# AKGWSB/EzRT

Measured on NVIDIA H100. Metric: Mrays/s (primary+secondary), higher is better.
Workload: dtype f32

## Files before the change

### ezrt_b200/csrc/device_functions.cuh

```cuda
#ifndef EZRT_DEVICE_FUNCTIONS_CUH
#define EZRT_DEVICE_FUNCTIONS_CUH

#include "device_scene.h"
#include "ezrt.h"
#include "ezrt_math.h"
#include "w8_node.h"

__constant__ uint32_t c_sobolV[8 * 32] = {
#include "ezrt_sobol_table.inc"
};

typedef ez_vec3 vec3;

__device__ __forceinline__ vec3 f4xyz(float4 q) { return ez_v3(q.x, q.y, q.z); }
__device__ __forceinline__ vec3 splat3(float s) { return ez_v3(s, s, s); }
__device__ __forceinline__ float4 ldg4(const float4* p) { return __ldg(p); }

#ifndef EZRT_MATH_NOINLINE
#define EZRT_MATH_NOINLINE 0
#endif
#if EZRT_MATH_NOINLINE
#define EZD_MATH __device__ __noinline__
#else
#define EZD_MATH __device__ __forceinline__
// ... 1146 lines not shown
                const unsigned p = __ballot_sync(FULL, member && da[a] >= 0.0f);
                signs |= (p == members ? 1u : (p == 0u ? 2u : 0u)) << (2 * a);
                const float4 b = make_float4(warp_reduce_f<0>(member ? oa[a] : INFINITY), warp_reduce_f<1>(member ? oa[a] : -INFINITY),
                                             warp_reduce_f<0>(member ? va[a] : INFINITY), warp_reduce_f<1>(member ? va[a] : -INFINITY));
                bnd[a] = b;
            }
        }
        const uint32_t near_mask = __shfl_sync(FULL, (d.x >= 0.0f ? (1u << sc.w8_near_bit[0]) : 0u) | (d.y >= 0.0f ? (1u << sc.w8_near_bit[1]) : 0u) |
                                                         (d.z >= 0.0f ? (1u << sc.w8_near_bit[2]) : 0u), __ffs(members) - 1);
        float L = EZ_INF;
        int sp = 0;
        uint32_t node = 0, g_base = 0, g_bits = 0;
        while (true) {
            const uint4* nd = nodes + (size_t)node * (W8_NODE_WORDS / 4);
            const uint4 h = ldg128_u32(nd), c = ldg128_u32(nd + 1), l = ldg128_u32(nd + 2), m = ldg128_u32(nd + 3), u = ldg128_u32(nd + 4);
            if (COUNT && lane == 0) ++*s_visits;
            bool hit = false;
            if (lane < 8) {
                const float sx = __uint_as_float(W8_SCALE_BITS(h.w, 0)), sy = __uint_as_float(W8_SCALE_BITS(h.w, 1)), sz = __uint_as_float(W8_SCALE_BITS(h.w, 2));
                const float ox = __uint_as_float(h.x), oy = __uint_as_float(h.y), oz = __uint_as_float(h.z);
                float ex, ey, ez, xx, xy, xz;
                w8_bundle_axis(__fadd_rd(ox, (slot_byte(c.z, c.w) - 0.25f) * sx), __fadd_ru(ox, (slot_byte(m.z, m.w) + 0.25f) * sx), signs & 3u, bnd[0], ex, xx);
                w8_bundle_axis(__fadd_rd(oy, (slot_byte(l.x, l.y) - 0.25f) * sy), __fadd_ru(oy, (slot_byte(u.x, u.y) + 0.25f) * sy), (signs >> 2) & 3u, bnd[1], ey, xy);
                w8_bundle_axis(__fadd_rd(oz, (slot_byte(l.z, l.w) - 0.25f) * sz), __fadd_ru(oz, (slot_byte(u.z, u.w) + 0.25f) * sz), signs >> 4, bnd[2], ez, xz);
                hit = fmaxf(fmaxf(ex, ey), fmaxf(ez, 0.0f)) <= fminf(fminf(xx, xy), fminf(xz, L));
            }
            const uint32_t hits = __ballot_sync(FULL, hit) & 0xffu;
            const uint32_t imask = h.w >> 24;
            const uint32_t inner = hits & imask;
            uint32_t leaf = hits & ~imask;
            if ((g_bits >> 8) != 0u) stack[sp++] = make_uint2(g_base, g_bits);
            g_base = c.x;
            g_bits = imask | ((uint32_t)s_perm[near_mask * 256u + inner] << 8);
            uint32_t t_mask = 0u;
            while (leaf != 0u) {
                const int s = __ffs(leaf) - 1;
                leaf &= leaf - 1u;
                const uint32_t mb = ((s < 4 ? m.x : m.y) >> ((s & 3) * 8)) & 0xffu;
                t_mask |= ((1u << (mb >> 5)) - 1u) << (mb & 31u);
            }
            if (t_mask != 0u) {
                while (t_mask != 0u) {
                    const int tri = (int)c.y + __ffs(t_mask) - 1;
                    t_mask &= t_mask - 1u;
                    if (member) {
                        if (COUNT) n_tests++;
                        float t = 0.0f;
                        const int r = IDX ? tri_test_idx_t<true>(sc.acc_tri_geo + (size_t)tri * 2, sc.acc_tri_vert, o, d, best, t, tri_na)
                                          : tri_test_t<true>(sc.acc_tri_geo + (size_t)tri * 4, o, d, best, t, tri_na);
                        if (r == 2) tie = true;
                        else if (r == 1) { best = t; best_tri = tri; tie = false; }
                    }
                }
                const float slack = sc.prune_delta * fmaxf(ez_abs(inv.x), fmaxf(ez_abs(inv.y), ez_abs(inv.z)));
                const float lim = member ? best + (best * 0.000244140625f + slack) : 0.0f;
                L = __uint_as_float(__reduce_max_sync(FULL, __float_as_uint(lim)));
            }
            if ((g_bits >> 8) == 0u) {
                if (sp == 0) break;
                const uint2 e = stack[--sp];
                g_base = e.x;
                g_bits = e.y;
            }
            const int p = 23 - __clz(g_bits);
            g_bits ^= 0x100u << p;
            const uint32_t slot = (uint32_t)p ^ near_mask;
            node = g_base + (uint32_t)__popc(g_bits & 0xffu & ((1u << slot) - 1u));
        }
        if (member) {
            HitRec hr;
            hr.t = best;
            hr.tri = best_tri;
            io.store(idx, hr, tie, o, d, inv);
        }
        }
    }
    if (COUNT) {
        if (lane == 0) atomicAdd(counts.node_visits, (unsigned long long)*s_visits);
        atomicAdd(counts.tri_tests, (unsigned long long)n_tests);
    }
}

struct MaterialDev {
    vec3 emissive, baseColor;
    float subsurface, metallic, specular, specularTint, roughness, anisotropic, sheen, sheenTint, clearcoat,
        clearcoatGloss;
};

__device__ __forceinline__ MaterialDev load_material(const SceneDev& sc, int matId) {
    const float4* m = sc.materials + (size_t)matId * 5;
    float4 a = ldg4(m), b = ldg4(m + 1), c = ldg4(m + 2), d = ldg4(m + 3);
    MaterialDev r;
    r.emissive = ez_v3(a.x, a.y, a.z);
    r.baseColor = ez_v3(a.w, b.x, b.y);
    r.subsurface = b.z; r.metallic = b.w; r.specular = c.x; r.specularTint = c.y;
    r.roughness = c.z; r.anisotropic = c.w; r.sheen = d.x; r.sheenTint = d.y;
    r.clearcoat = d.z; r.clearcoatGloss = d.w;
    return r;
}
__device__ __forceinline__ vec3 load_emissive(const SceneDev& sc, int matId) {
    float4 a = ldg4(sc.materials + (size_t)matId * 5);
    return ez_v3(a.x, a.y, a.z);
}

struct SurfaceHit {
    vec3 P, N;
    int matId;
    bool inside;
};

__device__ __forceinline__ const float4* tri_geo_rec(const SceneDev& sc, int tri, bool accel_space) {
    return accel_space ? sc.acc_tri_geo + (size_t)tri * (sc.acc_tri_indexed ? 2 : 4) : sc.tri_geo + (size_t)tri * 4;
}
__device__ __forceinline__ SurfaceHit surface_hit(const SceneDev& sc, vec3 o, vec3 d, float t, int tri, bool p3fudge, bool accel_space = false) {
    const float4* g = tri_geo_rec(sc, tri, accel_space);
    const float4* v = g;
    uint32_t i1 = 1u, i2 = 2u, i3 = 3u;
    if (accel_space && sc.acc_tri_indexed) {
        const uint4 qi = __ldg(reinterpret_cast<const uint4*>(g + 1));
        v = sc.acc_tri_vert; i1 = qi.x; i2 = qi.y; i3 = qi.z;
    }
    float4 q0 = ldg4(g), q1 = ldg4(v + i1), q2 = ldg4(v + i2), q3 = ldg4(v + i3);
    const float4* s = (accel_space ? sc.acc_tri_shade : sc.tri_shade) + (size_t)tri * 3;
    float4 m0 = ldg4(s), m1 = ldg4(s + 1), m2 = ldg4(s + 2);
    vec3 p1 = f4xyz(q1), p2 = f4xyz(q2), p3 = f4xyz(q3);
    vec3 Ng = f4xyz(q0);
    bool inside = ez_dot(Ng, d) > 0.0f;
    vec3 P = ez_add(o, ez_scale(d, t));
    float alpha, beta;
    float an = (-(P.x - p2.x)) * (p3.y - p2.y) + (P.y - p2.y) * (p3.x - p2.x);
    float bn = (-(P.x - p3.x)) * (p1.y - p3.y) + (P.y - p3.y) * (p1.x - p3.x);
    if (!p3fudge) {
        alpha = EZ_DIV(an, ((-(p1.x - p2.x)) * (p3.y - p2.y) + (p1.y - p2.y) * (p3.x - p2.x)) + 1e-7f);
        beta = EZ_DIV(bn, ((-(p2.x - p3.x)) * (p1.y - p3.y) + (p2.y - p3.y) * (p1.x - p3.x)) + 1e-7f);
    } else {
        alpha = EZ_DIV(an, (-((p1.x - p2.x) - 0.00005f)) * ((p3.y - p2.y) + 0.00005f) +
                               ((p1.y - p2.y) + 0.00005f) * ((p3.x - p2.x) + 0.00005f));
        beta = EZ_DIV(bn, (-((p2.x - p3.x) - 0.00005f)) * ((p1.y - p3.y) + 0.00005f) +
                              ((p2.y - p3.y) + 0.00005f) * ((p1.x - p3.x) + 0.00005f));
    }
    float gama = (1.0f - alpha) - beta;
    vec3 Ns = ez_add(ez_add(ez_scale(f4xyz(m0), alpha), ez_scale(f4xyz(m1), beta)), ez_scale(f4xyz(m2), gama));
    Ns = ez_normalize(Ns);
    SurfaceHit r;
    r.P = P;
    r.N = inside ? ez_neg(Ns) : Ns;
    r.matId = __float_as_int(m0.w);
    r.inside = inside;
    return r;
}
__device__ __forceinline__ int tri_material(const SceneDev& sc, int tri) {
    return __float_as_int(ldg4(sc.tri_shade + (size_t)tri * 3).w);
}

__device__ __forceinline__ float SchlickFresnel(float u) {
    float m = ez_clamp(1.0f - u, 0.0f, 1.0f);
    float m2 = m * m;
    return m2 * m2 * m;
}
__device__ __forceinline__ float GTR1(float NdotH, float a) {
    if (a >= 1.0f) return EZ_DIV(1.0f, EZ_PI);
    float a2 = a * a;
    float t = 1.0f + (a2 - 1.0f) * NdotH * NdotH;
    return EZ_DIV(a2 - 1.0f, EZ_PI * ezd_log(a2) * t);
}
__device__ __forceinline__ float GTR2(float NdotH, float a) {
    float a2 = a * a;
    float t = 1.0f + (a2 - 1.0f) * NdotH * NdotH;
    return EZ_DIV(a2, EZ_PI * t * t);
}
__device__ __forceinline__ float GTR2_aniso(float NdotH, float HdotX, float HdotY, float ax, float ay) {
    float s = ez_sqr(EZ_DIV(HdotX, ax)) + ez_sqr(EZ_DIV(HdotY, ay)) + NdotH * NdotH;
    return EZ_DIV(1.0f, EZ_PI * ax * ay * ez_sqr(s));
}
__device__ __forceinline__ float smithG_GGX(float NdotV, float alphaG) {
    float a = alphaG * alphaG;
    float b = NdotV * NdotV;
    return EZ_DIV(1.0f, NdotV + EZ_SQRT(a + b - a * b));
}
__device__ __forceinline__ float smithG_GGX_aniso(float NdotV, float VdotX, float VdotY, float ax, float ay) {
    return EZ_DIV(1.0f, NdotV + EZ_SQRT(ez_sqr(VdotX * ax) + ez_sqr(VdotY * ay) + ez_sqr(NdotV)));
}
__device__ __forceinline__ void get_tangent(vec3 N, vec3& tangent, vec3& bitangent) {
    vec3 helper = ez_v3(1.0f, 0.0f, 0.0f);
    if (ez_abs(N.x) > 0.999f) helper = ez_v3(0.0f, 0.0f, 1.0f);
    bitangent = ez_normalize(ez_cross(N, helper));
    tangent = ez_normalize(ez_cross(N, bitangent));
}

template <bool ANISO>
__device__ __forceinline__ vec3 brdf_evaluate(vec3 V, vec3 N, vec3 L, const MaterialDev& mat) {
    float NdotL = ez_dot(N, L);
    float NdotV = ez_dot(N, V);
    if (NdotL < 0.0f || NdotV < 0.0f) return splat3(0.0f);

    vec3 H = ez_normalize(ez_add(L, V));
    float NdotH = ez_dot(N, H);
    float LdotH = ez_dot(L, H);

    vec3 Cdlin = mat.baseColor;
    float Cdlum = 0.3f * Cdlin.x + 0.6f * Cdlin.y + 0.1f * Cdlin.z;
    vec3 Ctint = (Cdlum > 0.0f) ? ez_divs(Cdlin, Cdlum) : splat3(1.0f);
    vec3 Cspec = ez_scale(ez_vmix(splat3(1.0f), Ctint, mat.specularTint), mat.specular);
    vec3 Cspec0 = ez_vmix(ez_scale(Cspec, 0.08f), Cdlin, mat.metallic);
    vec3 Csheen = ez_vmix(splat3(1.0f), Ctint, mat.sheenTint);

    float Fd90 = 0.5f + 2.0f * LdotH * LdotH * mat.roughness;
    float FL = SchlickFresnel(NdotL);
    float FV = SchlickFresnel(NdotV);
    float Fd = ez_mix(1.0f, Fd90, FL) * ez_mix(1.0f, Fd90, FV);

    float Fss90 = LdotH * LdotH * mat.roughness;
    float Fss = ez_mix(1.0f, Fss90, FL) * ez_mix(1.0f, Fss90, FV);
    float ss = 1.25f * (Fss * (EZ_DIV(1.0f, NdotL + NdotV) - 0.5f) + 0.5f);

    float Ds, Gs;
    float FH = SchlickFresnel(LdotH);
    vec3 Fs = ez_vmix(Cspec0, splat3(1.0f), FH);
    if (!ANISO) {
        float alpha = ez_max(0.001f, ez_sqr(mat.roughness));
        Ds = GTR2(NdotH, alpha);
        Gs = smithG_GGX(NdotL, mat.roughness);
        Gs *= smithG_GGX(NdotV, mat.roughness);
    } else {
        vec3 X, Y;
        get_tangent(N, X, Y);
        float aspect = EZ_SQRT(1.0f - mat.anisotropic * 0.9f);
        float ax = ez_max(0.001f, EZ_DIV(ez_sqr(mat.roughness), aspect));
        float ay = ez_max(0.001f, ez_sqr(mat.roughness) * aspect);
        Ds = GTR2_aniso(NdotH, ez_dot(H, X), ez_dot(H, Y), ax, ay);
        Gs = smithG_GGX_aniso(NdotL, ez_dot(L, X), ez_dot(L, Y), ax, ay);
        Gs *= smithG_GGX_aniso(NdotV, ez_dot(V, X), ez_dot(V, Y), ax, ay);
    }

    float Dr = GTR1(NdotH, ez_mix(0.1f, 0.001f, mat.clearcoatGloss));
    float Fr = ez_mix(0.04f, 1.0f, FH);
    float Gr = smithG_GGX(NdotL, 0.25f) * smithG_GGX(NdotV, 0.25f);

    vec3 Fsheen = ez_scale(Csheen, FH * mat.sheen);
    vec3 diffuse = ez_add(ez_scale(Cdlin, EZ_DIV(1.0f, EZ_PI) * ez_mix(Fd, ss, mat.subsurface)), Fsheen);
    vec3 specular = ez_scale(ez_scale(Fs, Gs), Ds);
    vec3 clearcoat = splat3(0.25f * Gr * Fr * Dr * mat.clearcoat);
    return ez_add(ez_add(ez_scale(diffuse, 1.0f - mat.metallic), specular), clearcoat);
}

__device__ __forceinline__ float brdf_pdf(vec3 V, vec3 N, vec3 L, const MaterialDev& mat) {
    float NdotL = ez_dot(N, L);
    float NdotV = ez_dot(N, V);
    if (NdotL < 0.0f || NdotV < 0.0f) return 0.0f;
    vec3 H = ez_normalize(ez_add(L, V));
    float NdotH = ez_dot(N, H);
    float alpha = ez_max(0.001f, ez_sqr(mat.roughness));
    float Ds = GTR2(NdotH, alpha);
    float Dr = GTR1(NdotH, ez_mix(0.1f, 0.001f, mat.clearcoatGloss));
    float LH4 = 4.0f * ez_dot(L, H);
    float pdf_diffuse = EZ_DIV(NdotL, EZ_PI);
    float pdf_specular = EZ_DIV(Ds * NdotH, LH4);
    float pdf_clearcoat = EZ_DIV(Dr * NdotH, LH4);
    float r_diffuse = 1.0f - mat.metallic;
    float r_specular = 1.0f;
    float r_clearcoat = 0.25f * mat.clearcoat;
    float r_sum = r_diffuse + r_specular + r_clearcoat;
    float p_diffuse = EZ_DIV(r_diffuse, r_sum);
    float p_specular = EZ_DIV(r_specular, r_sum);
    float p_clearcoat = EZ_DIV(r_clearcoat, r_sum);
    float pdf = p_diffuse * pdf_diffuse + p_specular * pdf_specular + p_clearcoat * pdf_clearcoat;
    return ez_max(1e-10f, pdf);
}
__device__ __forceinline__ float mis_mix_weight(float a, float b) {
    float t = a * a;
    return EZ_DIV(t, b * b + t);
}

struct TransLobe {
    float t, eta, alpha;
    bool matched;
};
__device__ __forceinline__ TransLobe trans_lobe(const SceneDev& sc, int matId, const MaterialDev& mat, bool inside) {
    const float4 e = ldg4(sc.materials + (size_t)matId * 5 + 4);
    TransLobe r;
    r.t = ez_trans_weight(e.y, mat.metallic, e.x);
    r.eta = ez_trans_eta(e.x, inside);
    r.alpha = ez_max(0.001f, ez_sqr(mat.roughness));
    r.matched = ez_trans_matched(e.x) != 0;
    return r;
}
__device__ __forceinline__ vec3 bsdf_evaluate(vec3 V, vec3 N, vec3 L, const MaterialDev& mat, const TransLobe& tl, float& pdf) {
    vec3 f_ref = splat3(0.0f), f_diel = splat3(0.0f);
    float pdf_ref = 0.0f, pdf_diel = 0.0f;
    if (ez_dot(N, L) > 0.0f) { f_ref = brdf_evaluate<false>(V, N, L, mat); pdf_ref = brdf_pdf(V, N, L, mat); }
    if (!tl.matched) f_diel = ez_diel_eval(V, N, L, mat.baseColor, tl.alpha, tl.eta, &pdf_diel);
    return ez_trans_mix(f_ref, pdf_ref, f_diel, pdf_diel, tl.t, &pdf);
}

__device__ __forceinline__ vec3 to_normal_hemisphere(vec3 v, vec3 N) {
    vec3 helper = ez_v3(1.0f, 0.0f, 0.0f);
    if (ez_abs(N.x) > 0.999f) helper = ez_v3(0.0f, 0.0f, 1.0f);
    vec3 tangent = ez_normalize(ez_cross(N, helper));
    vec3 bitangent = ez_normalize(ez_cross(N, tangent));
    return ez_add(ez_add(ez_scale(tangent, v.x), ez_scale(bitangent, v.y)), ez_scale(N, v.z));
}
__device__ __forceinline__ vec3 sample_hemisphere(float xi_1, float xi_2) {
    float z = xi_1;
    float r = ez_max(0.0f, EZ_SQRT(1.0f - z * z));
    float phi = 2.0f * EZ_PI * xi_2;
    return ez_v3(r * ezd_cos(phi), r * ezd_sin(phi), z);
// ... 235 lines not shown
    const float4* r = (accel_space ? tex.acc_rec : tex.rec) + (size_t)tri * 2;
    const float4 a = ldg4(r), b = ldg4(r + 1);
    const int id = __float_as_int(b.z);
    const uint32_t maps = __float_as_uint(b.w);
    vec3 p1, p2, p3;
    tri_vertices(sc, tri, accel_space, p1, p2, p3);
    const vec3 Ng = f4xyz(ldg4(tri_geo_rec(sc, tri, accel_space)));
    float w1, w2, w3, u, v;
    ez_tri_bary(P, p1, p2, p3, Ng, &w1, &w2, &w3);
    const float uv6[6] = {a.x, a.y, a.z, a.w, b.x, b.y};
    ez_tex_uv(w1, w2, w3, uv6, &u, &v);
    if (uv_out) { uv_out[0] = u; uv_out[1] = v; }
    if (id >= 0) {
        const int4 t = __ldg(tex.table + id);
        mat.baseColor = ez_mul(mat.baseColor, ez_tex_sample(tex.texels + t.x, t.y, t.z, u, v, tex.lut));
    }
    const int mr = ez_maps_mr_id(maps), nm = ez_maps_normal_id(maps);
    if (mr >= 0) {
        const int4 t = __ldg(tex.table + mr);
        ez_mr_apply(ez_tex_sample(tex.texels + t.x, t.y, t.z, u, v, maps_dev.unorm), &mat.roughness, &mat.metallic);
    }
    if (nm >= 0) {
        const int4 t = __ldg(tex.table + nm);
        N = ez_normal_map(p1, p2, p3, uv6, u, v, ez_tex_sample(tex.texels + t.x, t.y, t.z, u, v, maps_dev.unorm), N, inside, V);
    }
}

template <bool AOV, bool ENV, bool TEX = false, bool MAPS = false>
__device__ __forceinline__ bool medium_step(const SceneDev& sc, const RenderDev& rd, int bounce, PathRegs& p, float t_s, float hit_t,
                                            int hit_tri, vec3& Lo, vec3& Le, bool& primary_miss, ShadowRay& sh, float4* aov_rec,
                                            const LightsDev& lights, const EnvDev& env, const MediumDev& med, const TexDev& tex = TexDev{},
                                            const MapsDev& maps = MapsDev{}) {
    if (bounce == 0) {
        Lo = splat3(0.0f);
        Le = splat3(0.0f);
        primary_miss = hit_tri < 0;
        if (AOV && hit_tri >= 0) {
            SurfaceHit hit = surface_hit(sc, p.o, p.d, hit_t, hit_tri, false, rd.accel_space != 0);
            MaterialDev mat = load_material(sc, hit.matId);
            if constexpr (MAPS) tex_material(sc, tex, maps, hit_tri, rd.accel_space != 0, hit.P, ez_neg(p.d), hit.inside, mat, hit.N);
            else if constexpr (TEX) mat.baseColor = tex_base_color(sc, tex, hit_tri, rd.accel_space != 0, hit.P, mat.baseColor);
            aov_rec[0] = make_float4(mat.baseColor.x, mat.baseColor.y, mat.baseColor.z, hit_t);
            aov_rec[1] = make_float4(hit.N.x, hit.N.y, hit.N.z, 0.0f);
        }
    } else {
        p.history = ez_mul(p.history, ez_divs(ez_scale(p.f_r, p.cosine_i), p.pdf));
    }
    p.history = ez_mul(p.history, med.albedo);
    if (bounce >= rd.max_bounce) return false;
    const vec3 P = ez_add(p.o, ez_scale(p.d, t_s));
    const float r_sel = rand01(p.seed);
    const float r_1 = rand01(p.seed);
    const float r_2 = rand01(p.seed);
    bool env_pick = false;
    float r_tri = r_sel;
    if constexpr (ENV) {
        const bool half = (env.p_env == 0.5f);
        env_pick = (env.p_env == 1.0f) || (half && r_sel < 0.5f);
        if (half) r_tri = (r_sel - 0.5f) * 2.0f;
        if (env_pick) {
            int texel;
            const vec3 Le_dir = ez_env_sample(env.row_cdf, env.col_cdf, env.w, env.h, r_1, r_2, &texel);
            const float pdf_e = env.p_env * ez_env_pdf(env.texel_pdf, env.w, env.h, Le_dir);
            if (ez_finite(pdf_e) && pdf_e > 0.0f) {
                sh.valid = true;
                sh.d = Le_dir;
                sh.tmax = EZ_INF;
                sh.pdf = pdf_e;
                sh.light_mat = -1;
            }
        }
    }
    if (!env_pick && lights.n > 0) {
        const float4* lr = lights.rec + 4 * (size_t)ez_light_select(lights.cdf, lights.n, r_tri);
        const float4 a = ldg4(lr), b = ldg4(lr + 1), c = ldg4(lr + 2), e = ldg4(lr + 3);
        const vec3 D = ez_sub(ez_triangle_point(f4xyz(a), f4xyz(b), f4xyz(c), r_1, r_2), P);
        const float dist = EZ_SQRT(ez_dot(D, D));
        const vec3 Ll = ez_normalize(D);
        const float cos_l = ez_abs(ez_dot(f4xyz(e), Ll));
        if (cos_l != 0.0f && dist != 0.0f) {
            sh.valid = true;
            sh.d = Ll;
            sh.tmax = ez_light_tmax(dist);
            sh.pdf = ez_light_pdf(e.w, lights.w_total, dist, cos_l);
            if constexpr (ENV) sh.pdf = sh.pdf * (1.0f - env.p_env);
            sh.light_mat = __float_as_int(a.w);
        }
    }
    if (sh.valid) {
        sh.o = P;
        sh.N = splat3(0.0f); sh.V = p.d; sh.history = p.history; sh.matId = EZRT_MEDIUM_VERTEX;
    }
    const float h_1 = rand01(p.seed);
    const float h_2 = rand01(p.seed);
    const vec3 L = ez_hg_sample(p.d, med.g, h_1, h_2);
    const float pdf = ez_hg_pdf(p.d, L, med.g);
    p.f_r = splat3(pdf);
    p.pdf = pdf;
    p.cosine_i = 1.0f;
    p.o = P;
    p.d = L;
    return true;
}

template <int MODE, bool DEFER_NEE = false, bool AOV = false, bool ENV = false, bool TRANS = false, bool MEDIUM = false, bool TEX = false,
          bool MAPS = false>
__device__ __forceinline__ bool shade_step(const SceneDev& sc, const RenderDev& rd, int bounce, PathRegs& p, float hit_t,
                                           int hit_tri, uint32_t px, uint32_t py, float2 sob, vec3& Lo, vec3& Le,
                                           bool& primary_miss, ShadowRay& sh, float4* aov_rec = nullptr, LightsDev lights = LightsDev{},
                                           EnvDev env = EnvDev{}, MediumDev med = MediumDev{}, TexDev tex = TexDev{}, vec3* sh_base = nullptr,
                                           float2* sh_rm = nullptr, MapsDev maps = MapsDev{}) {
    sh.valid = false;
    const int mode = (MODE < 0) ? rd.mode : MODE;
    const bool is_mode = (mode == EZRT_MODE_DISNEY_IS_MIS_P5);
    constexpr bool lights_mode = (MODE == EZRT_MODE_DISNEY_LIGHTS);
    const bool below = TRANS && p.cosine_i < 0.0f;
    static_assert(lights_mode || !TEX, "textures are rendered in the light sampling mode");
    static_assert(TEX || !MAPS, "material maps are rendered with the textures");
    if constexpr (MEDIUM) {
        static_assert(lights_mode && !TRANS, "the medium is rendered in the light sampling mode, without transmission");
        if (bounce > 0 && p.pdf <= 0.0f) return false;
        float t_s;
        const float t_end = (hit_tri < 0) ? __int_as_float(0x7f800000) : hit_t;
        if (ez_medium_flight(&med, p.o, p.d, t_end, &p.seed, &t_s))
            return medium_step<AOV, ENV, TEX, MAPS>(sc, rd, bounce, p, t_s, hit_t, hit_tri, Lo, Le, primary_miss, sh, aov_rec, lights, env, med, tex, maps);
    }
    if (bounce == 0) {
        Lo = splat3(0.0f);
        Le = splat3(0.0f);
        primary_miss = false;
        if (hit_tri < 0) {
            Lo = hdr_color(sc, rd, p.d, mode);
            primary_miss = true;
            return false;
        }
    } else {
        if ((is_mode || lights_mode) && p.pdf <= 0.0f) return false;
        if (hit_tri < 0) {
            vec3 sky = hdr_color(sc, rd, p.d, mode);
            if (is_mode) {
                float pdf_light = hdr_pdf(sc, p.d);
                float mis_weight = mis_mix_weight(p.pdf, pdf_light);
                vec3 c = ez_divs(ez_scale(ez_mul(ez_mul(ez_scale(p.history, mis_weight), sky), p.f_r), p.cosine_i), p.pdf);
                Lo = ez_add(Lo, c);
            } else if (ENV) {
                const float w = (env.p_env > 0.0f && !below) ? mis_mix_weight(p.pdf, env.p_env * ez_env_pdf(env.texel_pdf, env.w, env.h, p.d)) : 1.0f;
                Lo = ez_add(Lo, ez_divs(ez_scale(ez_mul(ez_mul(ez_scale(p.history, w), sky), p.f_r), path_cos<TRANS>(p.cosine_i)), p.pdf));
            } else {
                Lo = ez_add(Lo, contrib3(p.history, sky, p.f_r, path_cos<TRANS>(p.cosine_i), p.pdf));
            }
            return false;
        }
    }
    const bool fudge = (mode == EZRT_MODE_DIFFUSE_P3 || mode == EZRT_MODE_DISNEY_ANISO_P4);
    SurfaceHit hit = surface_hit(sc, p.o, p.d, hit_t, hit_tri, fudge, rd.accel_space != 0);
    MaterialDev mat = load_material(sc, hit.matId);
    if constexpr (TEX) {
        if ((AOV && bounce == 0) || bounce < rd.max_bounce) {
            if constexpr (MAPS) {
                tex_material(sc, tex, maps, hit_tri, rd.accel_space != 0, hit.P, ez_neg(p.d), hit.inside, mat, hit.N);
                *sh_rm = make_float2(mat.roughness, mat.metallic);
            } else {
                mat.baseColor = tex_base_color(sc, tex, hit_tri, rd.accel_space != 0, hit.P, mat.baseColor);
            }
            *sh_base = mat.baseColor;
        }
    }
    if (bounce == 0) {
        Le = mat.emissive;
        if (AOV) {
            aov_rec[0] = make_float4(mat.baseColor.x, mat.baseColor.y, mat.baseColor.z, hit_t);
            aov_rec[1] = make_float4(hit.N.x, hit.N.y, hit.N.z, 0.0f);
        }
    } else {
        if (lights_mode) {
            float w = 1.0f;
            const float lum = ez_luminance(mat.emissive);
            if (lum > 0.0f && !below) {
                vec3 p1, p2, p3;
                tri_vertices(sc, hit_tri, rd.accel_space != 0, p1, p2, p3);
                if (ez_is_light(ez_light_weight(p1, p2, p3, mat.emissive))) {
                    const vec3 Ng = f4xyz(ldg4(tri_geo_rec(sc, hit_tri, rd.accel_space != 0)));
                    if constexpr (ENV) w = mis_mix_weight(p.pdf, (1.0f - env.p_env) * ez_light_pdf(lum, lights.w_total, hit_t, ez_abs(ez_dot(Ng, p.d))));
                    else w = mis_mix_weight(p.pdf, ez_light_pdf(lum, lights.w_total, hit_t, ez_abs(ez_dot(Ng, p.d))));
                }
            }
            Lo = ez_add(Lo, ez_divs(ez_scale(ez_mul(ez_mul(ez_scale(p.history, w), mat.emissive), p.f_r), path_cos<TRANS>(p.cosine_i)), p.pdf));
        } else {
            Lo = ez_add(Lo, contrib3(p.history, mat.emissive, p.f_r, p.cosine_i, p.pdf));
        }
        p.history = ez_mul(p.history, ez_divs(ez_scale(p.f_r, path_cos<TRANS>(p.cosine_i)), p.pdf));
    }
    if (bounce >= rd.max_bounce) return false;

    vec3 V = ez_neg(p.d);
    vec3 N = hit.N;
    vec3 L;
    if (lights_mode) {
        const float r_sel = rand01(p.seed);
        const float r_1 = rand01(p.seed);
        const float r_2 = rand01(p.seed);
        float xi_1 = sob.x, xi_2 = sob.y;
        cp_rotate(xi_1, xi_2, px, py);
        const float xi_3 = rand01(p.seed);
        L = sample_brdf(xi_1, xi_2, xi_3, V, N, mat);
        float NdotL = ez_dot(N, L);
        vec3 fr_l = splat3(0.0f);
        float pdf_l = 0.0f;
        if (NdotL > 0.0f) { fr_l = brdf_evaluate<false>(V, N, L, mat); pdf_l = brdf_pdf(V, N, L, mat); }
        bool go = !(NdotL <= 0.0f);
        if constexpr (TRANS) {
            const TransLobe tl = trans_lobe(sc, hit.matId, mat, hit.inside);
            if (tl.t != 0.0f) go = bsdf_sample(xi_1, xi_2, xi_3, rand01(p.seed), V, N, mat, tl, L, fr_l, pdf_l, NdotL);
        }
        const int sh_mat = (TRANS && hit.inside) ? ~hit.matId : hit.matId;
        bool env_pick = false;
        float r_tri = r_sel;
        if constexpr (ENV) {
            const bool half = (env.p_env == 0.5f);
            env_pick = (env.p_env == 1.0f) || (half && r_sel < 0.5f);
            if (half) r_tri = (r_sel - 0.5f) * 2.0f;
            if (env_pick) {
                int texel;
                const vec3 Le_dir = ez_env_sample(env.row_cdf, env.col_cdf, env.w, env.h, r_1, r_2, &texel);
                const float pdf_e = env.p_env * ez_env_pdf(env.texel_pdf, env.w, env.h, Le_dir);
                if (ez_finite(pdf_e) && pdf_e > 0.0f && ez_dot(N, Le_dir) > 0.0f) {
                    sh.valid = true;
                    sh.o = hit.P;
                    sh.d = Le_dir;
                    sh.N = N; sh.V = V; sh.history = p.history; sh.matId = sh_mat;
                    sh.tmax = EZ_INF;
                    sh.pdf = pdf_e;
                    sh.light_mat = -1;
                }
            }
        }
        if (!env_pick && lights.n > 0) {
            const float4* lr = lights.rec + 4 * (size_t)ez_light_select(lights.cdf, lights.n, r_tri);
            const float4 a = ldg4(lr), b = ldg4(lr + 1), c = ldg4(lr + 2), e = ldg4(lr + 3);
            const int self = __float_as_int(rd.accel_space ? c.w : b.w);
            const vec3 D = ez_sub(ez_triangle_point(f4xyz(a), f4xyz(b), f4xyz(c), r_1, r_2), hit.P);
            const float dist = EZ_SQRT(ez_dot(D, D));
            const vec3 Ll = ez_normalize(D);
            const float cos_l = ez_abs(ez_dot(f4xyz(e), Ll));
            if (self != hit_tri && ez_dot(N, Ll) > 0.0f && cos_l != 0.0f && dist != 0.0f) {
                sh.valid = true;
                sh.o = hit.P;
                sh.d = Ll;
                sh.N = N; sh.V = V; sh.history = p.history; sh.matId = sh_mat;
                sh.tmax = ez_light_tmax(dist);
                sh.pdf = ez_light_pdf(e.w, lights.w_total, dist, cos_l);
                if constexpr (ENV) sh.pdf = sh.pdf * (1.0f - env.p_env);
                sh.light_mat = __float_as_int(a.w);
            }
        }
        if (!go) return false;
        p.f_r = fr_l;
        p.pdf = pdf_l;
        p.cosine_i = NdotL;
    } else if (is_mode) {
        float r1 = rand01(p.seed);
        float r2 = rand01(p.seed);
        float xi_1 = sob.x, xi_2 = sob.y;
        cp_rotate(xi_1, xi_2, px, py);
        float xi_3 = rand01(p.seed);
        const vec3 Lh = sample_hdr(sc, r1, r2);
        const float NdotLh = ez_dot(N, Lh);
        L = sample_brdf(xi_1, xi_2, xi_3, V, N, mat);
        const float NdotL = ez_dot(N, L);
        vec3 fr_l = splat3(0.0f);
        float pdf_l = 0.0f;
        if (NdotL > 0.0f) { fr_l = brdf_evaluate<false>(V, N, L, mat); pdf_l = brdf_pdf(V, N, L, mat); }
        if (NdotLh > 0.0f) {
            sh.valid = true;
            sh.o = hit.P;
            sh.d = Lh;
            if (DEFER_NEE) {
                sh.N = N; sh.V = V; sh.history = p.history; sh.matId = hit.matId;
            } else {
                sh.contrib = nee_contrib(sc, rd, mode, V, N, Lh, mat, p.history);
            }
        }
        if (NdotL <= 0.0f) return false;
        p.f_r = fr_l;
        p.pdf = pdf_l;
        p.cosine_i = NdotL;
    } else {
        vec3 Lh;
        if (mode == EZRT_MODE_DISNEY_SOBOL_P5) {
            float u = sob.x, v = sob.y;
            cp_rotate(u, v, px, py);
            Lh = sample_hemisphere(u, v);
        } else {
            float z = rand01(p.seed);
            float r = ez_max(0.0f, EZ_SQRT(1.0f - z * z));
            float phi = 2.0f * EZ_PI * rand01(p.seed);
            Lh = ez_v3(r * ezd_cos(phi), r * ezd_sin(phi), z);
        }
        L = to_normal_hemisphere(Lh, N);
        p.pdf = EZ_DIV(1.0f, 2.0f * EZ_PI);
        p.cosine_i = ez_max(0.0f, ez_dot(L, N));
        if (mode == EZRT_MODE_DIFFUSE_P3) p.f_r = ez_divs(mat.baseColor, EZ_PI);
        else if (mode == EZRT_MODE_DISNEY_ANISO_P4) p.f_r = brdf_evaluate<true>(V, N, L, mat);
        else p.f_r = brdf_evaluate<false>(V, N, L, mat);
    }
    p.o = hit.P;
    p.d = L;
    return true;
}

#endif
```

### ezrt_b200/csrc/kernels.cu

```cuda
#include "kernels.h"

#include <cstdlib>
#include <map>
#include <mutex>
#include <type_traits>

#include "device_functions.cuh"

__device__ __forceinline__ void in_tile_xy(int in_tile, int& ix, int& iy) {
    int sub = in_tile >> 5, lane = in_tile & 31;
    ix = (sub & 1) * 8 + (lane & 7);
    iy = (sub >> 1) * 4 + (lane >> 3);
}
__device__ __forceinline__ bool slot_pixel(const RenderDev& rd, const TileDev* __restrict__ tiles, uint32_t slot,
                                           uint32_t& px, uint32_t& py, uint32_t& frame_in_batch) {
    uint32_t per_frame = (uint32_t)rd.n_tiles * EZRT_TILE_PIXELS;
    frame_in_batch = slot / per_frame;
    uint32_t r = slot - frame_in_batch * per_frame;
    TileDev t = tiles[r >> 8];
    int ix, iy;
    in_tile_xy((int)(r & 255u), ix, iy);
    px = (uint32_t)(t.x0 + ix);
    py = (uint32_t)(t.y0 + iy);
    return ix < t.w && iy < t.h;
// ... 371 lines not shown
    uint2* stack_sm;
    w8_smem_setup(s_perm, stack_sm);
    AccelShadowIO io;
    io.base.sq = sq;
    io.base.Lo = Lo;
    io.base.perm = nullptr;
    io.acc_tri_leaf = sc.acc_tri_leaf;
    io.leaf_box = sc.leaf_box;
    io.defer_list = defer_list;
    io.defer_count = defer_count;
    extend_w8<true, COUNT, IDX, BOUNDED>(sc, *s_count, work, io, s_perm, stack_sm, counts, phase_cycles);
}

template <bool COUNT, bool Q16>
__global__ void __launch_bounds__(EZRT_EXTEND_MAX_THREADS, EZRT_EXTEND_LB_BLOCKS) k_extend_accel(SceneDev sc, PathQueue q, const uint32_t* __restrict__ q_count, uint32_t* work,
                                                                      uint32_t* defer_list, uint32_t* defer_count, W8Counts counts, const uint32_t* __restrict__ perm) {
    AccelExtendIO io;
    io.q = q;
    io.acc_tri_leaf = sc.acc_tri_leaf;
    io.leaf_box = sc.leaf_box;
    io.defer_list = defer_list;
    io.defer_count = defer_count;
    io.perm = perm;
    extend_persistent<true, false, true, true, 4, COUNT, Q16>(sc, accel_tree(sc), *q_count, work, io, g_smem_top, counts);
}
template <bool COUNT>
__global__ void __launch_bounds__(EZRT_EXTEND_MAX_THREADS, EZRT_EXTEND_LB_BLOCKS) k_extend_accel_camera(SceneDev sc, RenderDev rd, const TileDev* __restrict__ tiles,
                                                                      uint32_t batch_first_frame, uint32_t n_slots, uint32_t n_frames, PathQueue q, uint32_t* work,
                                                                      uint32_t* defer_list, uint32_t* defer_count, W8Counts counts) {
    AccelCameraIO io;
    io.rd = rd;
    io.tiles = tiles;
    io.batch_first_frame = batch_first_frame;
    io.n_frames = n_frames;
    io.per_frame = (uint32_t)rd.n_tiles * EZRT_TILE_PIXELS;
    io.q = q;
    io.acc_tri_leaf = sc.acc_tri_leaf;
    io.leaf_box = sc.leaf_box;
    io.defer_list = defer_list;
    io.defer_count = defer_count;
    extend_persistent<true, false, true, true, 4, COUNT, false>(sc, accel_tree(sc), n_slots, work, io, g_smem_top, counts, sc.refill_thresh_camera, sc.work_chunk_camera);
}
template <bool COUNT, bool Q16, bool BOUNDED = false>
__global__ void __launch_bounds__(EZRT_EXTEND_MAX_THREADS, EZRT_EXTEND_LB_BLOCKS) k_shadow_accel(SceneDev sc, ShadowQueue sq, const uint32_t* __restrict__ s_count, uint32_t* work,
                                                                      float4* __restrict__ Lo, uint32_t* defer_list, uint32_t* defer_count, W8Counts counts) {
    AccelShadowIO io;
    io.base.sq = sq;
    io.base.Lo = Lo;
    io.base.perm = nullptr;
    io.acc_tri_leaf = sc.acc_tri_leaf;
    io.leaf_box = sc.leaf_box;
    io.defer_list = defer_list;
    io.defer_count = defer_count;
    extend_persistent<true, true, true, true, 4, COUNT, Q16, BOUNDED>(sc, accel_tree(sc), *s_count, work, io, g_smem_top, counts);
}

#ifndef EZRT_SHADE_REGROUP
#define EZRT_SHADE_REGROUP 0
#endif
#define EZRT_SOBOL_TABLE 256
#define EZRT_SHADE_KEYS 18
#ifndef EZRT_SHADE_PREFETCH
#define EZRT_SHADE_PREFETCH 0
#endif
#ifndef EZRT_SHADE_MIN_BLOCKS
#define EZRT_SHADE_MIN_BLOCKS 8
#endif
template <int MODE, bool LIST, bool AOV = false, bool ENV = false, bool TRANS = false, bool MEDIUM = false, bool TEX = false,
          bool MAPS = false>
__global__ void __launch_bounds__(128, EZRT_SHADE_MIN_BLOCKS) k_shade(SceneDev sc, RenderDev rd, const TileDev* __restrict__ tiles, int bounce,
                                               uint32_t batch_first_frame, PathQueue qin, const uint32_t* __restrict__ in_count,
                                               PathQueue qout, uint32_t* out_count, ShadowQueue sq, uint32_t* s_count,
                                               float4* __restrict__ Lo, float4* __restrict__ Le, uint32_t n_fused, uint32_t n_frames,
                                               const uint32_t* __restrict__ list, const float2* __restrict__ side_hit,
                                               float4* __restrict__ aov_rec, LightsDev lights, EnvDev env, MediumDev med, TexDev tex,
                                               MapsDev maps) {
    __shared__ float2 s_sobol[EZRT_SOBOL_TABLE];
    const bool sobol_table = (MODE == EZRT_MODE_DISNEY_SOBOL_P5 || MODE == EZRT_MODE_DISNEY_IS_MIS_P5 || MODE == EZRT_MODE_DISNEY_LIGHTS) &&
                             n_frames <= EZRT_SOBOL_TABLE;
    if (sobol_table) {
        for (uint32_t f = threadIdx.x; f < n_frames; f += blockDim.x) s_sobol[f] = sobol_pair(bounce, batch_first_frame + f);
        __syncthreads();
    }
    __shared__ uint32_t s_scan[34];
    const uint32_t n = (LIST || !n_fused) ? *in_count : n_fused;
    if (LIST && n > EZRT_SIDE_CAP) return;
    const uint32_t n_round = ((n + blockDim.x - 1u) / blockDim.x) * blockDim.x;
    const uint32_t stride = gridDim.x * blockDim.x;
#if EZRT_SHADE_REGROUP
    __shared__ float4 s_rg[4][128];
    __shared__ float2 s_rg_hit[128];
    __shared__ unsigned short s_rg_cnt[4][2];
#endif
    for (uint32_t i0 = blockIdx.x * blockDim.x + threadIdx.x; i0 < n_round; i0 += stride) {
        uint32_t i = i0;
#if EZRT_SHADE_PREFETCH
        int next_tri = -1;
        if (!LIST && i0 + stride < n) next_tri = __float_as_int(__ldcs(qin.hit + i0 + stride).y);
#endif
        bool alive = false;
        PathRegs p;
        ShadowRay sh;
        sh.valid = false;
        vec3 sh_base;
        float2 sh_rm;
        uint32_t slot = 0;
        uint32_t px = 0, py = 0, fib = 0;
        bool present = i < n;
        float2 hit = make_float2(0.0f, 0.0f);
        float4 o4 = make_float4(0.0f, 0.0f, 0.0f, 0.0f), d4 = o4, h4 = o4, f4 = o4;
        bool staged = false;
#if EZRT_SHADE_REGROUP
        if (!LIST && bounce > 0) {
            staged = true;
            hit = make_float2(0.0f, __int_as_float(EZRT_TRI_PENDING));
            if (present) {
                hit = __ldcs(qin.hit + i);
                o4 = __ldcs(qin.ray_o + i); d4 = __ldcs(qin.ray_d + i); h4 = __ldcs(qin.hist + i); f4 = __ldcs(qin.fr + i);
            }
            const int tri0 = __float_as_int(hit.y);
            const int key = (tri0 == EZRT_TRI_PENDING) ? 2 : (tri0 >= 0 ? 0 : 1);
            const int lane = threadIdx.x & 31, wid = threadIdx.x >> 5;
            const unsigned lt = (1u << lane) - 1u;
            const unsigned m0 = __ballot_sync(0xffffffffu, key == 0), m1 = __ballot_sync(0xffffffffu, key == 1);
            if (lane == 0) { s_rg_cnt[wid][0] = (unsigned short)__popc(m0); s_rg_cnt[wid][1] = (unsigned short)__popc(m1); }
            __syncthreads();
            uint32_t n0 = 0, n1 = 0, b0 = 0, b1 = 0;
#pragma unroll
            for (int w = 0; w < 4; w++) {
                const uint32_t c0 = s_rg_cnt[w][0], c1 = s_rg_cnt[w][1];
                n0 += c0; n1 += c1;
                if (w < wid) { b0 += c0; b1 += c1; }
            }
            uint32_t dest;
            if (key == 0) dest = b0 + (uint32_t)__popc(m0 & lt);
            else if (key == 1) dest = n0 + b1 + (uint32_t)__popc(m1 & lt);
            else dest = n0 + n1 + ((uint32_t)wid * 32u - b0 - b1) + (uint32_t)__popc(~(m0 | m1) & lt);
            s_rg_hit[dest] = hit;
            s_rg[0][dest] = o4; s_rg[1][dest] = d4; s_rg[2][dest] = h4; s_rg[3][dest] = f4;
            __syncthreads();
            hit = s_rg_hit[threadIdx.x];
            o4 = s_rg[0][threadIdx.x]; d4 = s_rg[1][threadIdx.x]; h4 = s_rg[2][threadIdx.x]; f4 = s_rg[3][threadIdx.x];
            present = threadIdx.x < n0 + n1;
        }
#endif
        if (LIST && present) { hit = side_hit[i]; i = list[i]; }
        if (present && n_fused) present = slot_pixel(rd, tiles, i, px, py, fib);
        if (present) {
            if (!LIST && !staged) hit = __ldcs(qin.hit + i);
            if (n_fused) {
                slot = i;
                primary_ray(rd, px, py, batch_first_frame + fib, p.seed, p.o, p.d);
            } else {
                if (!staged) { o4 = __ldcs(qin.ray_o + i); d4 = __ldcs(qin.ray_d + i); }
                slot = __float_as_uint(d4.w);
                p.o = ez_v3(o4.x, o4.y, o4.z);
                p.d = ez_v3(d4.x, d4.y, d4.z);
                p.seed = __float_as_uint(o4.w);
                slot_pixel(rd, tiles, slot, px, py, fib);
            }
            vec3 lo = splat3(0.0f), le = splat3(0.0f);
            bool pmiss = false;
            float lo_w = 0.0f;
            if (bounce > 0) {
                if (!staged) { h4 = __ldcs(qin.hist + i); f4 = __ldcs(qin.fr + i); }
                p.history = ez_v3(h4.x, h4.y, h4.z);
                p.cosine_i = h4.w;
                p.f_r = ez_v3(f4.x, f4.y, f4.z);
                p.pdf = f4.w;
                float4 l4 = Lo[slot];
                lo = ez_v3(l4.x, l4.y, l4.z);
                lo_w = l4.w;
            } else {
                p.history = splat3(1.0f);
                p.f_r = splat3(0.0f);
                p.cosine_i = 0.0f;
                p.pdf = 1.0f;
            }
            const float2 sob = sobol_table ? s_sobol[fib] : sobol_pair(bounce, batch_first_frame + fib);
#if EZRT_SHADE_PREFETCH
            if (!LIST && next_tri >= 0) {
                const float4* g = tri_geo_rec(sc, next_tri, rd.accel_space != 0);
                const float4* sr = (rd.accel_space ? sc.acc_tri_shade : sc.tri_shade) + (size_t)next_tri * 3;
                asm volatile("prefetch.global.L2 [%0];" ::"l"(g));
                if (!(rd.accel_space && sc.acc_tri_indexed)) asm volatile("prefetch.global.L2 [%0];" ::"l"(g + 2));
                asm volatile("prefetch.global.L2 [%0];" ::"l"(sr));
                asm volatile("prefetch.global.L2 [%0];" ::"l"(sr + 2));
            }
#endif
            if (LIST || __float_as_int(hit.y) != EZRT_TRI_PENDING) {
                alive = shade_step<MODE, MODE == EZRT_MODE_DISNEY_IS_MIS_P5, AOV, ENV, TRANS, MEDIUM, TEX, MAPS>(sc, rd, bounce, p, hit.x, __float_as_int(hit.y), px, py,
                                                                                                          sob, lo, le, pmiss, sh, AOV ? aov_rec + 2 * (size_t)slot : nullptr,
                                                                                                          lights, env, med, tex, &sh_base, &sh_rm, maps);
                if (bounce == 0) {
                    lo_w = pmiss ? 1.0f : 0.0f;
                    if (le.x != 0.0f || le.y != 0.0f || le.z != 0.0f) {
                        Le[slot] = make_float4(le.x, le.y, le.z, 0.0f);
                        lo_w = 2.0f;
                    }
                }
                Lo[slot] = make_float4(lo.x, lo.y, lo.z, lo_w);
            }
        }
        uint32_t pos = block_append(alive, out_count, s_scan);
        if (alive) {
            __stcs(qout.ray_o + pos, make_float4(p.o.x, p.o.y, p.o.z, __uint_as_float(p.seed)));
            __stcs(qout.ray_d + pos, make_float4(p.d.x, p.d.y, p.d.z, __uint_as_float(slot)));
            __stcs(qout.hist + pos, make_float4(p.history.x, p.history.y, p.history.z, p.cosine_i));
            __stcs(qout.fr + pos, make_float4(p.f_r.x, p.f_r.y, p.f_r.z, p.pdf));
        }
        if (MODE == EZRT_MODE_DISNEY_IS_MIS_P5 || MODE == EZRT_MODE_DISNEY_LIGHTS) {
            constexpr bool LT = (MODE == EZRT_MODE_DISNEY_LIGHTS);
            uint32_t spos = block_append(sh.valid, s_count, s_scan);
            if (sh.valid) {
                __stcs(sq.ray_o + spos, make_float4(sh.o.x, sh.o.y, sh.o.z, __uint_as_float(slot)));
                __stcs(sq.ray_d + spos, make_float4(sh.d.x, sh.d.y, sh.d.z, __int_as_float(sh.matId)));
                __stcs(sq.nrm + spos, make_float4(sh.N.x, sh.N.y, sh.N.z, LT ? sh.tmax : 0.0f));
                __stcs(sq.view + spos, make_float4(sh.V.x, sh.V.y, sh.V.z, LT ? sh.pdf : 0.0f));
                __stcs(sq.hist + spos, make_float4(sh.history.x, sh.history.y, sh.history.z, LT ? __int_as_float(sh.light_mat) : 0.0f));
                if constexpr (TEX) {
                    if (sh.matId != EZRT_MEDIUM_VERTEX || !MEDIUM) {
                        __stcs(tex.sh_base + spos, make_float4(sh_base.x, sh_base.y, sh_base.z, MAPS ? sh_rm.x : 0.0f));
                        if constexpr (MAPS) __stcs(maps.sh_metal + spos, sh_rm.y);
                    }
                }
            }
        }
    }
}

template <int MODE, bool ENV = false, bool TRANS = false, bool MEDIUM = false, bool TEX = false, bool MAPS = false>
__global__ void __launch_bounds__(128, 8) k_nee(SceneDev sc, RenderDev rd, ShadowQueue sq, const uint32_t* __restrict__ s_count, float4* __restrict__ Lo,
                                                MediumDev med, TexDev tex, MapsDev maps) {
    static_assert(MODE == EZRT_MODE_DISNEY_LIGHTS || !(ENV || TRANS || MEDIUM), "the options exist in the light sampling mode");
    static_assert(!(TRANS && MEDIUM), "the medium is rendered without transmission");
    __shared__ uint32_t s_scan[34];
    __shared__ uint32_t s_total;
    __shared__ uint32_t s_list[512];
    const uint32_t n = *s_count;
    for (uint32_t base = blockIdx.x * 512u; base < n; base += gridDim.x * 512u) {
        if (threadIdx.x == 0) s_total = 0u;
        __syncthreads();
#pragma unroll 1
        for (int k = 0; k < 4; k++) {
            const uint32_t j = base + (uint32_t)k * 128u + threadIdx.x;
            const bool lit = j < n && sq.lit[j] != 0;
            const uint32_t pos = block_append(lit, &s_total, s_scan);
            if (lit) s_list[pos] = j;
        }
        __syncthreads();
        const uint32_t total = s_total;
        for (uint32_t q = threadIdx.x; q < total; q += blockDim.x) {
            const uint32_t j = s_list[q];
            const float4 o4 = __ldcs(sq.ray_o + j), d4 = __ldcs(sq.ray_d + j), n4 = __ldcs(sq.nrm + j), v4 = __ldcs(sq.view + j), h4 = __ldcs(sq.hist + j);
            const uint32_t slot = __float_as_uint(o4.w);
            const int m_raw = __float_as_int(d4.w);
            const auto material = [&](int m_id) {
                MaterialDev m = load_material(sc, m_id);
                if constexpr (MAPS) {
                    const float4 b = __ldcs(tex.sh_base + j);
                    m.baseColor = f4xyz(b);
                    m.roughness = b.w;
                    m.metallic = __ldcs(maps.sh_metal + j);
                } else if constexpr (TEX) {
                    m.baseColor = f4xyz(__ldcs(tex.sh_base + j));
                }
                return m;
            };
            const vec3 V = ez_v3(v4.x, v4.y, v4.z), N = ez_v3(n4.x, n4.y, n4.z), Ld = ez_v3(d4.x, d4.y, d4.z), hist = ez_v3(h4.x, h4.y, h4.z);
            vec3 c;
            if constexpr (MODE == EZRT_MODE_DISNEY_LIGHTS) {
                const int lm = __float_as_int(h4.w);
                const auto light_color = [&] { return (ENV && lm < 0) ? hdr_color(sc, rd, Ld, EZRT_MODE_DISNEY_LIGHTS) : load_emissive(sc, lm); };
                if constexpr (MEDIUM) {
                    const vec3 E = light_color();
                    if (m_raw == EZRT_MEDIUM_VERTEX) c = nee_medium_contrib(V, Ld, med.g, hist, E, v4.w);
                    else c = nee_light_contrib(V, N, Ld, material(m_raw), hist, E, v4.w);
                    c = ez_scale(c, ez_medium_transmittance(&med, ez_v3(o4.x, o4.y, o4.z), Ld, ez_medium_light_dist(n4.w, ENV && lm < 0)));
                } else {
                    const int m_id = (TRANS && m_raw < 0) ? ~m_raw : m_raw;
                    const MaterialDev mat = material(m_id);
                    if constexpr (TRANS) c = nee_trans_contrib(sc, V, N, Ld, m_id, mat, m_raw < 0, hist, light_color(), v4.w);
                    else c = nee_light_contrib(V, N, Ld, mat, hist, light_color(), v4.w);
                }
            } else {
                c = nee_contrib(sc, rd, EZRT_MODE_DISNEY_IS_MIS_P5, V, N, Ld, load_material(sc, m_raw), hist);
            }
            float4 lo = Lo[slot];
            lo.x += c.x; lo.y += c.y; lo.z += c.z;
            Lo[slot] = lo;
        }
        __syncthreads();
    }
}

__device__ __forceinline__ size_t fb_index(const RenderDev& rd, const TileDev& t, int ix, int iy) {
    if (rd.compact_out) return (size_t)t.pixel_offset + (size_t)iy * t.w + ix;
    return (size_t)(t.y0 + iy) * rd.width + (t.x0 + ix);
}

template <bool ADAPTIVE, bool AOV = false>
__global__ void __launch_bounds__(256) k_blend(RenderDev rd, const TileDev* __restrict__ tiles, int nf, uint32_t batch_first_frame,
                                               const float4* __restrict__ Lo, const float4* __restrict__ Le, float* __restrict__ fb,
                                               float* __restrict__ luma2, int32_t* __restrict__ spp_map,
                                               const float4* __restrict__ aov_rec, float* __restrict__ aov) {
    uint32_t per_frame = (uint32_t)rd.n_tiles * EZRT_TILE_PIXELS;
    uint32_t r = blockIdx.x * blockDim.x + threadIdx.x;
    if (r >= per_frame) return;
    TileDev t = tiles[r >> 8];
    int ix, iy;
    in_tile_xy((int)(r & 255u), ix, iy);
    if (ix >= t.w || iy >= t.h) return;
    const size_t pix = fb_index(rd, t, ix, iy);
    size_t idx = pix * (size_t)rd.out_channels;
    const bool fresh = (batch_first_frame == 0u) && (rd.first_frame == 0u);
    vec3 acc = fresh ? splat3(0.0f) : ez_v3(fb[idx], fb[idx + 1], fb[idx + 2]);
    float m2 = 0.0f;
    if (ADAPTIVE && !fresh) m2 = luma2[pix];
    float feat[8];
    if (AOV) {
#pragma unroll
        for (int k = 0; k < 8; k++) feat[k] = fresh ? 0.0f : aov[pix * 8 + k];
    }
    for (int f = 0; f < nf; f++) {
        float4 lo = Lo[(size_t)f * per_frame + r];
        vec3 color = ez_v3(lo.x, lo.y, lo.z);
        if (lo.w == 2.0f) {
            float4 le = Le[(size_t)f * per_frame + r];
            color = ez_add(ez_v3(le.x, le.y, le.z), color);
        }
        float a = EZ_DIV(1.0f, __uint2float_rn(batch_first_frame + (uint32_t)f + 1u));
        acc = ez_vmix(acc, color, a);
        if (ADAPTIVE) {
            const float y = ez_luminance(color);
            m2 = ez_mix(m2, y * y, a);
        }
        if (AOV) {
            float4 r0 = make_float4(0.0f, 0.0f, 0.0f, 0.0f), r1 = r0;
            float cov = 0.0f;
            if (lo.w != 1.0f) {
                const size_t s = (size_t)f * per_frame + r;
                r0 = aov_rec[2 * s];
                r1 = aov_rec[2 * s + 1];
                cov = 1.0f;
            }
            const float v[8] = {r0.x, r0.y, r0.z, cov, r1.x, r1.y, r1.z, r0.w};
#pragma unroll
            for (int k = 0; k < 8; k++) feat[k] = ez_mix(feat[k], v[k], a);
        }
    }
    fb[idx] = acc.x; fb[idx + 1] = acc.y; fb[idx + 2] = acc.z;
    if (rd.out_channels == 4) fb[idx + 3] = 1.0f;
    if (ADAPTIVE) luma2[pix] = m2;
    if (ADAPTIVE && !AOV) spp_map[pix] = (int32_t)(batch_first_frame + (uint32_t)nf);
// ... 669 lines not shown
```

Measured before the change: 3515.

## Skip full shading at last bounce and make Lo accumulation read-modify-write only when nonzero

```diff
diff --git a/ezrt_b200/csrc/device_functions.cuh b/ezrt_b200/csrc/device_functions.cuh
--- a/ezrt_b200/csrc/device_functions.cuh
+++ b/ezrt_b200/csrc/device_functions.cuh
@@ -1322,6 +1322,9 @@
 __device__ __forceinline__ int tri_material(const SceneDev& sc, int tri) {
     return __float_as_int(ldg4(sc.tri_shade + (size_t)tri * 3).w);
 }
+__device__ __forceinline__ int hit_material(const SceneDev& sc, int tri, bool accel_space) {
+    return __float_as_int(ldg4((accel_space ? sc.acc_tri_shade : sc.tri_shade) + (size_t)tri * 3).w);
+}
 
 __device__ __forceinline__ float SchlickFresnel(float u) {
     float m = ez_clamp(1.0f - u, 0.0f, 1.0f);
@@ -1863,6 +1866,28 @@
             return false;
         }
     }
+    const auto add_emission = [&](vec3 E) {
+        if (lights_mode) {
+            float w = 1.0f;
+            const float lum = ez_luminance(E);
+            if (lum > 0.0f && !below) {
+                vec3 p1, p2, p3;
+                tri_vertices(sc, hit_tri, rd.accel_space != 0, p1, p2, p3);
+                if (ez_is_light(ez_light_weight(p1, p2, p3, E))) {
+                    const vec3 Ng = f4xyz(ldg4(tri_geo_rec(sc, hit_tri, rd.accel_space != 0)));
+                    if constexpr (ENV) w = mis_mix_weight(p.pdf, (1.0f - env.p_env) * ez_light_pdf(lum, lights.w_total, hit_t, ez_abs(ez_dot(Ng, p.d))));
+                    else w = mis_mix_weight(p.pdf, ez_light_pdf(lum, lights.w_total, hit_t, ez_abs(ez_dot(Ng, p.d))));
+                }
+            }
+            Lo = ez_add(Lo, ez_divs(ez_scale(ez_mul(ez_mul(ez_scale(p.history, w), E), p.f_r), path_cos<TRANS>(p.cosine_i)), p.pdf));
+        } else {
+            Lo = ez_add(Lo, contrib3(p.history, E, p.f_r, p.cosine_i, p.pdf));
+        }
+    };
+    if (bounce > 0 && bounce >= rd.max_bounce) {
+        add_emission(load_emissive(sc, hit_material(sc, hit_tri, rd.accel_space != 0)));
+        return false;
+    }
     const bool fudge = (mode == EZRT_MODE_DIFFUSE_P3 || mode == EZRT_MODE_DISNEY_ANISO_P4);
     SurfaceHit hit = surface_hit(sc, p.o, p.d, hit_t, hit_tri, fudge, rd.accel_space != 0);
     MaterialDev mat = load_material(sc, hit.matId);
@@ -1884,22 +1909,7 @@
             aov_rec[1] = make_float4(hit.N.x, hit.N.y, hit.N.z, 0.0f);
         }
     } else {
-        if (lights_mode) {
-            float w = 1.0f;
-            const float lum = ez_luminance(mat.emissive);
-            if (lum > 0.0f && !below) {
-                vec3 p1, p2, p3;
-                tri_vertices(sc, hit_tri, rd.accel_space != 0, p1, p2, p3);
-                if (ez_is_light(ez_light_weight(p1, p2, p3, mat.emissive))) {
-                    const vec3 Ng = f4xyz(ldg4(tri_geo_rec(sc, hit_tri, rd.accel_space != 0)));
-                    if constexpr (ENV) w = mis_mix_weight(p.pdf, (1.0f - env.p_env) * ez_light_pdf(lum, lights.w_total, hit_t, ez_abs(ez_dot(Ng, p.d))));
-                    else w = mis_mix_weight(p.pdf, ez_light_pdf(lum, lights.w_total, hit_t, ez_abs(ez_dot(Ng, p.d))));
-                }
-            }
-            Lo = ez_add(Lo, ez_divs(ez_scale(ez_mul(ez_mul(ez_scale(p.history, w), mat.emissive), p.f_r), path_cos<TRANS>(p.cosine_i)), p.pdf));
-        } else {
-            Lo = ez_add(Lo, contrib3(p.history, mat.emissive, p.f_r, p.cosine_i, p.pdf));
-        }
+        add_emission(mat.emissive);
         p.history = ez_mul(p.history, ez_divs(ez_scale(p.f_r, path_cos<TRANS>(p.cosine_i)), p.pdf));
     }
     if (bounce >= rd.max_bounce) return false;
diff --git a/ezrt_b200/csrc/kernels.cu b/ezrt_b200/csrc/kernels.cu
--- a/ezrt_b200/csrc/kernels.cu
+++ b/ezrt_b200/csrc/kernels.cu
@@ -547,7 +547,10 @@
                 slot = i;
                 primary_ray(rd, px, py, batch_first_frame + fib, p.seed, p.o, p.d);
             } else {
-                if (!staged) { o4 = __ldcs(qin.ray_o + i); d4 = __ldcs(qin.ray_d + i); }
+                if (!staged) {
+                    if (MEDIUM || bounce == 0 || bounce < rd.max_bounce) o4 = __ldcs(qin.ray_o + i);
+                    d4 = __ldcs(qin.ray_d + i);
+                }
                 slot = __float_as_uint(d4.w);
                 p.o = ez_v3(o4.x, o4.y, o4.z);
                 p.d = ez_v3(d4.x, d4.y, d4.z);
@@ -563,15 +566,16 @@
                 p.cosine_i = h4.w;
                 p.f_r = ez_v3(f4.x, f4.y, f4.z);
                 p.pdf = f4.w;
-                float4 l4 = Lo[slot];
-                lo = ez_v3(l4.x, l4.y, l4.z);
-                lo_w = l4.w;
             } else {
                 p.history = splat3(1.0f);
                 p.f_r = splat3(0.0f);
                 p.cosine_i = 0.0f;
                 p.pdf = 1.0f;
             }
+            constexpr bool LO_EARLY = MODE != EZRT_MODE_DISNEY_IS_MIS_P5 && MODE != EZRT_MODE_DISNEY_LIGHTS;
+            float4 l4 = make_float4(0.0f, 0.0f, 0.0f, 0.0f);
+            const bool lo_early = LO_EARLY && bounce > 0 && __float_as_int(hit.y) == -1;
+            if (lo_early) l4 = Lo[slot];
             const float2 sob = sobol_table ? s_sobol[fib] : sobol_pair(bounce, batch_first_frame + fib);
 #if EZRT_SHADE_PREFETCH
             if (!LIST && next_tri >= 0) {
@@ -593,8 +597,12 @@
                         Le[slot] = make_float4(le.x, le.y, le.z, 0.0f);
                         lo_w = 2.0f;
                     }
+                    Lo[slot] = make_float4(lo.x, lo.y, lo.z, lo_w);
+                } else if (((__float_as_uint(lo.x) | __float_as_uint(lo.y) | __float_as_uint(lo.z)) & 0x7fffffffu) != 0u) {
+                    if (!lo_early) l4 = Lo[slot];
+                    l4.x += lo.x; l4.y += lo.y; l4.z += lo.z;
+                    Lo[slot] = l4;
                 }
-                Lo[slot] = make_float4(lo.x, lo.y, lo.z, lo_w);
             }
         }
         uint32_t pos = block_append(alive, out_count, s_scan);
```

After: 3533 (median of 6 runs). Within noise of the previous version (+0.5%).
